# mehtas30/Software-Defined-Radio-Course-Project

Hardware: NVIDIA B200
Metric: input IQ Msamples/s (mode 0 stereo) (higher is better)
Workload: dtype f32

## Files before the change

### software-defined-radio-course-project_b200/csrc/fmrx_kernels.cu

```cuda
#include <cstddef>
#include <mutex>
#include <type_traits>

#include "fmrx_internal.h"
#ifdef FMRX_PLL_PROFILE
#include <cstdio>
#endif

namespace fmrx {

constexpr int kMaxDevices = 64;
struct DeviceCfg {
    size_t rf_smem[2][3] = {};
    size_t audio_smem = 0;
    size_t bp_smem = 0;
    size_t pll_ring_only = 0, pll_whole_sm = 0;
    int sm_count = 0;
};
static std::mutex g_cfg_mutex;
static DeviceCfg g_cfg[kMaxDevices];
static DeviceCfg *device_cfg()
{
    int dev = -1;
    if (cudaGetDevice(&dev) != cudaSuccess || dev < 0 || dev >= kMaxDevices)
// ... 722 lines not shown
        int2 v;
        asm volatile("ld.shared.v2.b32 {%0, %1}, [%2];" : "=r"(v.x), "=r"(v.y) : "r"(addr));
        return v;
    };
    auto load_half = [&](unsigned addr) {
        int4 v;
        asm volatile("ld.volatile.shared.v4.b32 {%0, %1, %2, %3}, [%4];" : "=r"(v.x), "=r"(v.y), "=r"(v.z), "=r"(v.w) : "r"(addr) : "memory");
        return v;
    };
    auto settle = [&](int u0, int nb, float integ0, float ph0, int gi0) -> bool {
        if (guards_failed()) {
#ifdef FMRX_PLL_PROFILE
            r.prof_stamp += bad != 0;
            r.prof_c += bad == 0;
            if (bad == 0) {
                if (!(cmax < 1e30f)) r.prof_inv++;
                else if (cmax > 0.5f) r.prof_range++;
                else r.prof_tie++;
            }
#endif
            r.kbase = kbase;
            r.integ = integ0;
            r.ph = ph0;
            r.gi = gi0;
            n_exact++;
            if (!pll_block_exact(r, u0, nb, lane)) {
#ifdef FMRX_PLL_PROFILE
                r.prof_fatal_exact++;
                if (blockIdx.x == 0 && lane == 0)
                    printf("pll dbg fatal: group base %d block at %d (of %d) gi %d kbase %d\n", base, u0 - base, cnt, r.gi, r.kbase);
                __syncwarp();
#endif
                return false;
            }
            integ = r.integ;
            ph = r.ph;
            kpe = r.kpe;
            kie = r.kie;
            gi = r.gi;
        }
        bad = 0;
        cmax = 0.0f;
        return true;
    };
    auto load_rec = [&](int u) {
        int2 v;
        asm volatile("ld.volatile.shared.v2.b32 {%0, %1}, [%2];" : "=r"(v.x), "=r"(v.y) : "r"(sph_base + (unsigned)(u & (PLL_PH_RING - 1)) * 8u) : "memory");
        return v;
    };
    float pi_next = 0.0f;
    int kbase_next = 0, seq_next = 0;
    auto next_pi = [&](int u0) {
        const bool have = seq_next == u0 && fabsf(pi_next) < 2097152.0f;
        pi_f = have ? pi_next : pi_f;
        kbase = have ? kbase_next : kbase;
        bad |= (int)!have;
    };
    int t = 0;
    int fatal = 0;
    const int n_full = cnt >> 4;
    if (r.cont) {
        const int2 rec = load_rec(base - 1);
        block_pi(__int_as_float(rec.x), inv_ulp_f, pi_next, kbase_next);
        seq_next = rec.y;
    } else {
        pi_next = pi_f;
        kbase_next = kbase;
        seq_next = base;
    }
    for (int b = 0; b < n_full; b++, t += 16) {
        const int u0 = base + t;
        next_pi(u0);
        asm volatile("st.shared.b32 [%0], %1;" ::"r"(kb_base + 4u * (unsigned)(t >> 4)), "r"(kbase) : "memory");
        const float integ0 = integ, ph0 = ph;
        const int gi0 = gi;
        integ = p_faddf(integ, kie);
        ph = p_faddf(ph, p_faddf(kpe, integ));
        const unsigned in_a0 = in_base + (unsigned)(u0 & (PLL_RING - 1)) * (unsigned)sizeof(PllIn);
        const unsigned tab_a0 = tab_base + (unsigned)(u0 & (PLL_TABLES - 1)) * (unsigned)sizeof(PllRow);
        const int stamp = pll_stamp(u0, kbase);
        int gis[16];
        int4 rb0 = load_half(tab_a0 + 16u), ra0 = load_half(tab_a0);
        int4 rb1 = load_half(tab_a0 + (unsigned)sizeof(PllRow) + 16u), ra1 = load_half(tab_a0 + (unsigned)sizeof(PllRow));
        const int2 vg_last = load_vg(in_a0 + 15u * (unsigned)sizeof(PllIn));
#pragma unroll
        for (int j = 0; j < 16; j++) {
            int4 rb2 = rb1, ra2 = ra1;
            if (j + 2 < 16) {
                rb2 = load_half(tab_a0 + (unsigned)(j + 2) * (unsigned)sizeof(PllRow) + 16u);
                ra2 = load_half(tab_a0 + (unsigned)(j + 2) * (unsigned)sizeof(PllRow));
            }
            gis[j] = step(ra0, rb0, stamp, j == 15);
            ra0 = ra1; rb0 = rb1;
            ra1 = ra2; rb1 = rb2;
            if (j == 8) {
                const int2 rec = load_rec(u0 + 15);
                block_pi(__int_as_float(rec.x), inv_ulp_f, pi_next, kbase_next);
                seq_next = rec.y;
            }
        }
        gi = vg_last.x + kbase + __float_as_int(p_faddf(p_faddf(__int_as_float(gis[15]), __int_as_float(vg_last.y)), 12582912.0f));
#pragma unroll
        for (int j = 0; j < 16; j += 4)
            asm volatile("st.shared.v4.b32 [%0], {%1, %2, %3, %4};" ::"r"(sg_base + 4u * (unsigned)(t + j)), "r"(gis[j]), "r"(gis[j + 1]),
                         "r"(gis[j + 2]), "r"(gis[j + 3])
                         : "memory");
        if (!settle(u0, 16, integ0, ph0, gi0)) {
            fatal = 2;
            break;
        }
        if (n_exact > PLL_EXACT_MAX) {
            fatal = 1;
            break;
        }
        asm volatile("st.volatile.shared.b32 [%0], %1;" ::"r"(prog_addr), "r"(u0 + 16) : "memory");
    }
    if (!fatal && t < cnt) {
        const int u0 = base + t, nb = cnt - t;
        next_pi(u0);
        asm volatile("st.shared.b32 [%0], %1;" ::"r"(kb_base + 4u * (unsigned)(t >> 4)), "r"(kbase) : "memory");
        const float integ0 = integ, ph0 = ph;
        const int gi0 = gi;
        integ = p_faddf(integ, kie);
        ph = p_faddf(ph, p_faddf(kpe, integ));
        for (int j = 0; j < nb; j++) {
            const int u = u0 + j;
            const unsigned row = tab_base + (unsigned)(u & (PLL_TABLES - 1)) * (unsigned)sizeof(PllRow);
            const int4 rb = load_half(row + 16u), ra = load_half(row);
            const int2 vg = load_vg(in_base + (unsigned)(u & (PLL_RING - 1)) * (unsigned)sizeof(PllIn));
            const int tb = step(ra, rb, pll_stamp(u0, kbase), j == nb - 1);
            gi = vg.x + kbase + __float_as_int(p_faddf(p_faddf(__int_as_float(tb), __int_as_float(vg.y)), 12582912.0f));
            asm volatile("st.shared.b32 [%0], %1;" ::"r"(sg_base + 4u * (unsigned)(t + j)), "r"(tb) : "memory");
        }
        fatal = settle(u0, nb, integ0, ph0, gi0) ? 0 : 2;
    }
    r.fatal = fatal;
    r.t_stop = t;
    r.n_exact = n_exact;
    if (fatal == 2)
        return;
    r.integ = integ;
    r.ph = ph;
    r.kpe = kpe;
    r.kie = kie;
    r.gi = gi;
}

__global__ void __launch_bounds__(PLL_THREADS) k_pll(const PllArgs a)
{
    using namespace pllcore;
    extern __shared__ __align__(16) unsigned char pll_dyn_smem[];
    PllIn *s_in = reinterpret_cast<PllIn *>(pll_dyn_smem);
    __shared__ __align__(16) int2 s_ph[PLL_PH_RING];
    __shared__ float s_hdr[3];
    __shared__ double s_hdr_tad;
    __shared__ int s_kbase;
    __shared__ int s_kb_blk[2][PLL_GROUP / 16];
    __shared__ int s_prog;
    __shared__ PllRow s_tab[PLL_TABLES];
    __shared__ __align__(16) int s_g[2][PLL_GROUP];
    __shared__ double s_grid[2];
    __shared__ double s_prep_ulp[2];
    __shared__ int s_head_ready[PLL_IO_WARPS];
    __shared__ double s_ulp_hist[2];
    __shared__ int s_spec[2];
    __shared__ int s_split[2];
    __shared__ int s_flag[5];
    __shared__ int s_redo;

    const int c = blockIdx.x;
    const int warp = threadIdx.x >> 5, lane = threadIdx.x & 31;
    const float *p = a.pilot + (size_t)c * a.pilot_stride;
    float *tr = a.trig + (size_t)c * a.if_stride + a.if_off;
    float *st = a.state + 8 * (size_t)c;
    const int n = a.n_if;

    Consts k;
    k.kp = a.prm.kp;
    k.ki = a.prm.ki;
    k.w = a.prm.w;
    const TrigK &K = a.kconst;

    const float toff0 = st[5];
    const bool regular = toff_is_regular(toff0);
    const int t0 = regular ? (int)toff0 : 0;
    const int role = warp & 3;
    const int io_id = warp >> 2;
    const int cand_id = (warp >> 2) * 2 + role - 2;

    auto prepare_one = [&](int u, float e_slope, float e_ph, int e_base) {
        {
            const float pvv = (u < n) ? p[u] : 1.0f;
            const float pnx = (u + 1 < n) ? p[u + 1] : 1.0f;
            PllIn in;
            in.x = pvv;
            in.inv_x = 1.0 / (double)pvv;
            const float toff = (float)min(t0 + u + 1, 16777216);
            in.v = __dmul_rn(k.w, (double)toff);
            const double qv = grid_round(in.v, s_grid[1]);
            in.vi = grid_index(qv);
            in.vr = __double2float_rn(__fma_rn(in.v, s_grid[1], -p_add(qv, -FMRX_RINT_MAGIC)));
            in.c3 = predictor_c(k, pvv, (float)min(t0 + u, 16777216));
            in.h1 = onehyp_inputs(in.v, e_ph, e_slope, u + 1 - e_base, pnx);
            s_in[u & (PLL_RING - 1)] = in;
        }
    };
    auto prepare = [&](int base, float e_slope, float e_ph, int e_base) {
        for (int j = 32 * io_id; j < PLL_GROUP; j += 32 * PLL_IO_WARPS)
            prepare_one(base + j + lane, e_slope, e_ph, e_base);
        if (lane == 0 && io_id == 0)
            s_prep_ulp[(base / PLL_GROUP) & 1] = s_grid[0];
    };
    auto head_ready = [&](int next_base) -> bool {
        for (int spin = 0; spin < PLL_SPIN_LIMIT; spin++) {
            int a0, a1;
            asm volatile("ld.volatile.shared.b32 %0, [%1];" : "=r"(a0) : "r"(smem_u32(&s_head_ready[0])) : "memory");
            asm volatile("ld.volatile.shared.b32 %0, [%1];" : "=r"(a1) : "r"(smem_u32(&s_head_ready[1])) : "memory");
            if (a0 == next_base && a1 == next_base)
                return true;
        }
        return false;
    };

    for (int i = threadIdx.x; i < PLL_PH_RING; i += PLL_THREADS)
        s_ph[i] = make_int2(0, 0);
    for (int i = threadIdx.x; i < PLL_TABLES; i += PLL_THREADS) {
        s_tab[i].lp = PLL_ROW_INVALID;
        s_tab[i].stamp = 0;
        s_tab[i].kie0 = 0.0f;
    }
    if (threadIdx.x == 0) {
        s_flag[1] = 0;
        s_redo = 0;
        s_head_ready[0] = s_head_ready[1] = -1;
    }
    Chain ch;
    bool stale = false;
    bool have_ed = false;
    float kpe_next = 0.0f, kie_next = 0.0f;
    bool dead = false;
    int backoff = 0, skip = 0;
    int prev_scheme = 0;
    float ph_hdr_prev = 0.0f;
    int n_groups = 0, n_redone = 0, n_exact = 0, prev_exact = 0;
    float pred_integ = 0.0f, pred_ph = 0.0f;
#ifdef FMRX_PLL_PROFILE
    long long prof_steps_cyc = 0, prof_wait = 0, prof_pre = 0, prof_one_cyc = 0;
    long long prof_t_end = 0, prof_bar2 = 0, prof_hdr = 0, prof_bar1 = 0, prof_post = 0, prof_post2 = 0, prof_c1 = 0;
    const long long prof_k0 = clock64();
    int prof_steps = 0, prof_n_stamp = 0, prof_n_c = 0, prof_n_fe = 0, prof_n_fm = 0;
    int prof_n_tie = 0, prof_n_range = 0, prof_n_inv = 0;
    int prof_one_steps = 0, prof_one_groups = 0, prof_one_exact = 0, prof_one_short = 0, prof_checked = 0;
    __shared__ int s_prof[8];
    __shared__ long long s_prof1[8];
    if (threadIdx.x < 8) {
        s_prof[threadIdx.x] = 0;
        s_prof1[threadIdx.x] = 0;
    }
#endif
    if (warp == 0) {
        ch.integ = st[0];
        ch.ph = st[1];
        ch.fi = st[2];
        ch.fq = st[3];
        ch.toff = toff0;
        chain_load(ch, k);
        if (lane == 0) {
            s_grid[0] = ch.ulp;
            s_grid[1] = ch.inv_ulp;
        }
    }
    __syncthreads();
    if (role == 1 && io_id < PLL_IO_WARPS) {
        prepare(0, st[0], st[1], 0);
    }
    __syncthreads();

    for (int base = 0, g = 0; base < n;) {
        const int cnt = min(PLL_GROUP, n - base);
        Chain ck;
#ifdef FMRX_PLL_PROFILE
        const long long prof_h0 = clock64();
        if (warp == 0 && prof_t_end)
            prof_bar2 += prof_h0 - prof_t_end;
#endif
        if (warp == 0) {
            ck = ch;
            const bool again = s_redo != 0;
            const bool usable = regular && !dead && ch.binade != FMRX_DISARMED && fabs(ch.tad) <= (double)FMRX_FAST_TRIG_MAX;
            const bool can3 = usable && !again && skip == 0 && (double)fabsf(ch.ph) < ch.ulp * 16777216.0;
            const bool regrid = can3 && s_prep_ulp[g & 1] != ch.ulp;
            const int scheme = can3 ? 3 : usable ? 1 : 0;
            const bool cont = scheme == 3 && prev_scheme == 3 && have_ed && prev_exact <= 2 && !regrid;
#ifdef FMRX_PLL_PROFILE
            prof_post += clock64() - prof_h0;
#endif
            if (scheme != prev_scheme || again) {
                for (int i = lane; i < PLL_TABLES; i += 32) {
                    s_tab[i].lp = PLL_ROW_INVALID;
                    s_tab[i].stamp = 0;
                    s_tab[i].kie0 = 0.0f;
                }
                for (int i = lane; i < PLL_PH_RING; i += 32)
                    s_ph[i] = make_int2(0, 0);
            } else if (scheme == 3 && !cont && base > 0) {
                for (int i = lane; i < PLL_HEAD; i += 32) {
                    s_tab[(base + i) & (PLL_TABLES - 1)].lp = PLL_ROW_INVALID;
                    s_tab[(base + i) & (PLL_TABLES - 1)].stamp = 0;
                    s_ph[(base + i) & (PLL_PH_RING - 1)] = make_int2(0, 0);
                }
            }
            if (lane == 0) {
                s_flag[0] = scheme;
                s_flag[2] = regrid;
                s_grid[0] = ch.ulp;
                s_grid[1] = ch.inv_ulp;
                s_flag[3] = cont;
                s_flag[4] = again;
                s_kbase = __float_as_int(p_faddf(p_fmulf(ch.ph, (float)ch.inv_ulp), 12582912.0f)) - 0x4B400000 - 0x4B400000;
                s_hdr[0] = ch.integ;
                s_hdr[1] = ch.ph;
                if (!again) {
                    s_hdr[2] = g > 0 ? p_fmulf(p_faddf(ch.ph, -ph_hdr_prev), 1.0f / PLL_GROUP) : ch.integ;
                    ph_hdr_prev = ch.ph;
                }
                s_hdr_tad = ch.tad;
                s_prog = base;
            }
        }
#ifdef FMRX_PLL_PROFILE
        const long long prof_h1 = clock64();
#endif
        __syncthreads();
#ifdef FMRX_PLL_PROFILE
        if (warp == 0) {
            prof_hdr += prof_h1 - prof_h0;
            prof_bar1 += clock64() - prof_h1;
        }
#endif
        if (s_flag[2]) {
            const double iu = s_grid[1];
            for (int j = threadIdx.x; j < PLL_GROUP; j += PLL_THREADS) {
                PllIn &in = s_in[(base + j) & (PLL_RING - 1)];
                const double qv = grid_round(in.v, iu);
                in.vi = grid_index(qv);
                in.vr = __double2float_rn(__fma_rn(in.v, iu, -p_add(qv, -FMRX_RINT_MAGIC)));
            }
            if (threadIdx.x == 0)
                s_prep_ulp[g & 1] = s_grid[0];
            __syncthreads();
        }
        const int scheme = s_flag[0];
        const bool spec = scheme == 3;
        const bool again = s_flag[4] != 0;
        const double ulp = s_grid[0], inv_ulp = s_grid[1];
#ifdef FMRX_PLL_PROFILE
        const long long prof_ga = clock64();
#endif

        if (warp == 0) {
            if (lane == 0)
                s_redo = 0;
            if (!again)
                n_groups++;
            bool good = scheme != 0;
            bool redo = false;
            bool regridded = false;
            int split = 0;
            int parked = 0;
            if (scheme == 3) {
                float integ = ch.integ, ph = ch.ph;
                float kpe = kpe_next, kie = kie_next;
                if (!have_ed) {
                    const PllIn i0 = s_in[base & (PLL_RING - 1)];
                    const Feedback f0 = make_feedback(K, ch.tad, pll_turn(i0.x), i0.inv_x, nullptr, nullptr);
                    const float ed = error_from_feedback(f0, i0.x, (double)i0.x, good);
                    kpe = p_fmulf(k.kp, ed);
                    kie = p_fmulf(k.ki, ed);
                }
                const float inv_ulp_f = (float)inv_ulp;
                float pi_f = 0.0f;
                int cu_base = 0;
                auto recentre = [&]() {
                    const float pm = p_faddf(p_fmulf(ph, inv_ulp_f), 12582912.0f);
                    pi_f = p_faddf(pm, -12582912.0f);
                    cu_base = __float_as_int(pm) - 0x4B400000 - 0x4B400000;
                    good &= fabsf(pi_f) < 2097152.0f;
                };
                recentre();
#ifdef FMRX_PLL_PROFILE
                const long long prof_w0 = clock64();
                prof_pre += prof_w0 - prof_ga;
#endif
                {
                    const bool need = lane < 16 && lane < cnt;
                    int spin = 0;
                    for (;;) {
                        const int z = ld_v4(&s_tab[(base + (lane & 15)) & (PLL_TABLES - 1)].kpe2).w;
                        if (__all_sync(0xffffffffu, !need || (z & 0x3ffffff) == base + 1) || ++spin >= PLL_SPIN_LIMIT)
                            break;
                    }
                    if (spin >= PLL_SPIN_LIMIT) {
                        dead = true;
                        good = false;
                        if (lane == 0)
                            s_flag[1] = 1;
                    }
                }
#ifdef FMRX_PLL_PROFILE
                prof_wait += clock64() - prof_w0;
#endif
                TableRun r;
                r.integ = integ;
                r.ph = ph;
                r.kpe = kpe;
                r.kie = kie;
                r.inv_ulp_f = inv_ulp_f;
                r.pi_f = pi_f;
                r.kbase = cu_base;
                r.base = base;
                r.cnt = cnt;
                r.in_base = smem_u32(&s_in[0]) + (unsigned)offsetof(PllIn, vi);
                r.tab_base = smem_u32(&s_tab[0]);
                r.sg_base = smem_u32(&s_g[g & 1][0]);
                r.prog_addr = smem_u32(&s_prog);
                r.sph_base = smem_u32(&s_ph[0]);
                r.kb_base = smem_u32(&s_kb_blk[g & 1][0]);
                r.head_addr = smem_u32(&s_head_ready[0]);
                r.cont = s_flag[3];
#ifdef FMRX_PLL_PROFILE
                r.prof_stamp = r.prof_c = r.prof_fatal_exact = 0;
                r.prof_tie = r.prof_range = r.prof_inv = 0;
#endif
                r.gi = __double2int_rn(p_mul(ch.tad, inv_ulp));
                r.n_exact = 0;
                r.fatal = 0;
                r.ring = s_in;
                r.k = k;
                r.ulp = ulp;
                r.toff_base = ch.toff;
                if (good) {
                    __syncwarp();
#ifdef FMRX_PLL_PROFILE
                    const long long prof_c0 = clock64();
#endif
                    pll_table_group(r, lane);
#ifdef FMRX_PLL_PROFILE
                    prof_c1 = clock64();
                    prof_steps_cyc += prof_c1 - prof_c0;
                    prof_steps += cnt;
                    prof_n_stamp += r.prof_stamp;
                    prof_n_c += r.prof_c;
                    prof_n_fe += r.prof_fatal_exact;
                    prof_n_tie += r.prof_tie;
                    prof_n_range += r.prof_range;
                    prof_n_inv += r.prof_inv;
                    prof_n_fm += r.fatal && !r.prof_fatal_exact;
#endif
                    good = r.fatal == 0;
                    n_exact += r.n_exact;
                    prev_exact = r.n_exact;
                }
                if (good && r.fatal == 0)
                    split = cnt;
                if (r.fatal == 2) {
                    asm volatile("st.volatile.shared.b32 [%0], %1;" ::"r"(smem_u32(&s_prog)), "r"(PLL_ABANDONED) : "memory");
                    split = r.t_stop;
                    onehyp_chain_at(ch, r.integ, r.ph, (float)min(t0 + base + r.t_stop, 16777216), p_mul((double)r.gi, ulp));
                    pll_group_checked(ch, k, s_in, base, r.t_stop, cnt, regular, smem_u32(&s_g[g & 1][0]), false);
                    stale = false;
                    have_ed = false;
                    parked = 1;
                    regridded = true;
                } else if (good) {
                    ch.integ = r.integ;
                    ch.ph = r.ph;
                    ch.toff = (float)min(t0 + base + cnt, 16777216);
                    ch.tad = p_mul((double)r.gi, ulp);
                    stale = true;
                    have_ed = true;
                    kpe_next = r.kpe;
                    kie_next = r.kie;
                    backoff = 0;
                    parked = 1;
                } else {
                    asm volatile("st.volatile.shared.b32 [%0], %1;" ::"r"(smem_u32(&s_prog)), "r"(PLL_ABANDONED) : "memory");
                    n_redone++;
                    backoff = min(backoff < 4 ? backoff + 1 : 2 * backoff, PLL_BACKOFF_MAX);
                    skip = backoff;
                    ch = ck;
                    have_ed = false;
                    redo = !dead;
                    if (!redo) {
                        if (stale) {
                            chain_refresh(ch);
                            stale = false;
                        }
                        pll_group_checked(ch, k, s_in, base, 0, cnt, regular, smem_u32(&s_g[g & 1][0]), false);
                    }
                }
            } else if (scheme == 1) {
                if (skip > 0 && !again)
                    skip--;
                OneRun r;
                r.integ = ch.integ;
                r.ph = ch.ph;
                r.base = base;
                r.cnt = cnt;
                r.tab_base = smem_u32(&s_tab[0]);
                r.sg_base = smem_u32(&s_g[g & 1][0]);
                r.prog_addr = smem_u32(&s_prog);
                r.ring = s_in;
                r.k = k;
                r.toff_base = ch.toff;
                r.tad0 = ch.tad;
                r.n_exact = 0;
                r.done = 0;
                r.timed_out = 0;
                __syncwarp();
#ifdef FMRX_PLL_PROFILE
                const long long prof_c0 = clock64();
#endif
                pll_onehyp_group(r, lane);
#ifdef FMRX_PLL_PROFILE
                prof_one_cyc += clock64() - prof_c0;
                prof_one_steps += r.done;
                prof_one_groups++;
                prof_one_exact += r.n_exact;
                prof_one_short += r.done < cnt;
#endif
                n_exact += r.n_exact;
                if (r.timed_out) {
                    dead = true;
                    if (lane == 0)
                        s_flag[1] = 1;
                }
                const int last = base + r.done - 1;
                const double tad = r.done ? onehyp_trigarg(s_in[last & (PLL_RING - 1)].v, r.ph) : ch.tad;
                if (r.done < cnt) {
                    asm volatile("st.volatile.shared.b32 [%0], %1;" ::"r"(smem_u32(&s_prog)), "r"(PLL_ABANDONED) : "memory");
                    onehyp_chain_at(ch, r.integ, r.ph, (float)min(t0 + base + r.done, 16777216), tad);
                    pll_group_checked(ch, k, s_in, base, r.done, cnt, regular, smem_u32(&s_g[g & 1][0]), true);
                    stale = false;
                } else {
                    ch.integ = r.integ;
                    ch.ph = r.ph;
                    ch.toff = (float)min(t0 + base + cnt, 16777216);
                    ch.tad = tad;
                    stale = true;
                    if (fabs(tad) <= (double)FMRX_FAST_TRIG_MAX)
                        chain_arm(ch);
                    else
                        onehyp_chain_at(ch, r.integ, r.ph, ch.toff, tad), stale = false;
                }
                have_ed = false;
                parked = 2;
            } else {
                if (skip > 0)
                    skip--;
                if (stale) {
                    chain_refresh(ch);
                    stale = false;
                }
#ifdef FMRX_PLL_PROFILE
                prof_checked++;
#endif
                pll_group_checked(ch, k, s_in, base, 0, cnt, regular, smem_u32(&s_g[g & 1][0]), false);
                have_ed = false;
                parked = 0;
            }
            prev_scheme = redo || regridded ? 0 : scheme;
            if (lane == 0) {
                s_spec[g & 1] = parked;
                s_split[g & 1] = split;
                s_ulp_hist[g & 1] = ulp;
                s_redo = redo;
            }
#ifdef FMRX_PLL_PROFILE
            prof_t_end = clock64();
            if (prof_c1)
                prof_post2 += prof_t_end - prof_c1;
            prof_c1 = 0;
#endif
        } else if (role >= 2) {
            if (scheme == 3) {
                const int sq = lane >> 2, jq = lane & 3;
                const unsigned prog_a = smem_u32(&s_prog);
                auto progress = [&]() {
                    int v;
                    asm volatile("ld.volatile.shared.b32 %0, [%1];" : "=r"(v) : "r"(prog_a) : "memory");
                    return v;
                };
                const bool cont = s_flag[3] != 0;
                const int first = base + (cont ? PLL_HEAD : 0);
                const int end = base + cnt + (base + cnt + PLL_HEAD <= n ? PLL_HEAD : 0);
                const int q0 = first / PLL_BATCH;
                bool head_seen = false;
                for (int ub8 = first + ((cand_id - q0 % PLL_CAND_WARPS + PLL_CAND_WARPS) % PLL_CAND_WARPS) * PLL_BATCH; ub8 < end;
                     ub8 += PLL_BATCH * PLL_CAND_WARPS) {
                    if (!head_seen && cnt == PLL_GROUP && ub8 + PLL_BATCH >= base + cnt) {
                        if (!head_ready(base + PLL_GROUP)) {
                            s_flag[1] = 1;
                            break;
                        }
                        head_seen = true;
                    }
                    const bool live = ub8 + sq < end;
                    const int u = ub8 + (live ? sq : 0);
                    const double v = s_in[u & (PLL_RING - 1)].v;
                    const int vi = s_in[u & (PLL_RING - 1)].vi;
                    const float vr = s_in[u & (PLL_RING - 1)].vr;
                    const PllIn nx = s_in[(u + 1) & (PLL_RING - 1)];
                    const int last = min(ub8 + PLL_BATCH - 1, end - 1);
                    int prog = 0, spin = 0;
                    for (;; spin++) {
                        const int seq = ld_v2(&s_ph[last & (PLL_PH_RING - 1)]).y;
                        if (seq - (last + 1) >= 0 || spin >= PLL_SPIN_LIMIT)
                            break;
                        if ((spin & 7) == 7 && (prog = progress()) == PLL_ABANDONED)
                            break;
                    }
                    if (prog == PLL_ABANDONED)
                        break;
                    if (spin >= PLL_SPIN_LIMIT) {
                        s_flag[1] = 1;
                        break;
                    }
                    const int2 pr = ld_v2(&s_ph[u & (PLL_PH_RING - 1)]);
                    const int ub = ub8 & ~15;
                    int kb = s_kbase;
                    bool have_pi = true;
                    if (ub != base || cont) {
                        const int2 rb = ld_v2(&s_ph[(ub - 1) & (PLL_PH_RING - 1)]);
                        float pif;
                        block_pi(__int_as_float(rb.x), (float)inv_ulp, pif, kb);
                        have_pi = rb.y == ub;
                    }
                    const bool have = pr.y == u + 1 && have_pi;
                    const int gc = grid_index(grid_round(p_add(v, (double)__int_as_float(pr.x)), inv_ulp));
                    const int gl = gc - 1 + jq;
                    const double tad = p_mul((double)gl, ulp);
                    const Feedback f = make_feedback(K, tad, pll_turn(nx.x), nx.inv_x, nullptr, nullptr);
                    const int ag = gl < 0 ? -gl : gl;
                    bool ok = have && ag > (1 << 23) && ag < (1 << 24);
#ifdef FMRX_PLL_PROFILE
                    const bool prof_ok_b = ok;
#endif
                    const float ed = error_from_feedback(f, nx.x, (double)nx.x, ok);
                    const int n1 = gc - (vi + kb) - 0x4B400000;
#ifdef FMRX_PLL_PROFILE
                    if (live && jq < 3 && blockIdx.x == 0) {
                        if (!(pr.y == u + 1)) atomicAdd(&s_prof[0], 1);
                        else if (!have_pi) atomicAdd(&s_prof[1], 1);
                        else if (!prof_ok_b) atomicAdd(&s_prof[2], 1);
                        else if (!ok) atomicAdd(&s_prof[fabs(f.phi) >= FMRX_SEAM_PHI_MAX ? 3 : 4], 1);
                        else if (!(n1 >= -60 && n1 <= 60)) atomicAdd(&s_prof[5], 1);
                        else atomicAdd(&s_prof[6], 1);
                    }
#endif
                    ok = ok && n1 >= -60 && n1 <= 60;
                    const unsigned oks = __ballot_sync(0xffffffffu, ok || jq == 3);
                    const bool valid = ((oks >> (4 * sq)) & 7u) == 7u;
                    for (spin = 0; (prog = progress()) != PLL_ABANDONED && prog - (ub8 + PLL_BATCH - PLL_TABLES) < 0 && spin < PLL_SPIN_LIMIT;
                         spin++)
                        ;
                    if (prog == PLL_ABANDONED)
                        break;
                    if (spin >= PLL_SPIN_LIMIT) {
                        s_flag[1] = 1;
                        break;
                    }
                    if (live && prog - (ub8 + PLL_BATCH) < 0) {
                        const int lo = jq < 3 ? __float_as_int(p_fmulf(k.kp, ed))
                                              : __float_as_int(valid ? p_faddf(p_faddf((float)n1, -0.5f), -vr) : PLL_ROW_INVALID);
                        const int hi = jq < 3 ? __float_as_int(p_fmulf(k.ki, ed)) : pll_stamp(u & ~15, kb);
                        asm volatile("st.volatile.shared.v2.b32 [%0], {%1, %2};" ::"r"(smem_u32(&s_tab[u & (PLL_TABLES - 1)]) + 8u * (unsigned)jq),
                                     "r"(lo), "r"(hi)
                                     : "memory");
                    }
                }
            } else if (scheme == 1) {
                const unsigned prog_a = smem_u32(&s_prog);
                auto progress = [&]() {
                    int v;
                    asm volatile("ld.volatile.shared.b32 %0, [%1];" : "=r"(v) : "r"(prog_a) : "memory");
                    return v;
                };
                const int end = base + cnt;
                for (int ub = base + cand_id * PLL_BATCH1; ub < end; ub += PLL_BATCH1 * PLL_CAND_WARPS) {
                    const bool live = ub + lane < end;
                    const int u = live ? ub + lane : end - 1;
                    const int last = min(ub + PLL_BATCH1 - 1, end - 1);
                    int prog = 0, spin = 0;
#ifdef FMRX_PLL_PROFILE
                    const long long cw0 = clock64();
#endif
                    for (;; spin++) {
                        const int seq = ld_v2(&s_ph[last & (PLL_PH_RING - 1)]).y;
                        if (seq == last + 1 || spin >= PLL_SPIN_LIMIT)
                            break;
                        if ((spin & 7) == 7 && (prog = progress()) == PLL_ABANDONED)
                            break;
                    }
                    if (prog == PLL_ABANDONED)
                        break;
                    if (spin >= PLL_SPIN_LIMIT) {
                        s_flag[1] = 1;
                        break;
                    }
#ifdef FMRX_PLL_PROFILE
                    const long long cw1 = clock64();
#endif
                    const int2 cur = ld_v2(&s_ph[u & (PLL_PH_RING - 1)]);
                    bool ok = cur.y == u + 1;
                    double tad = s_hdr_tad;
                    if (u != base) {
                        const int2 prv = ld_v2(&s_ph[(u - 1) & (PLL_PH_RING - 1)]);
                        ok = ok && prv.y == u;
                        tad = onehyp_trigarg(s_in[(u - 1) & (PLL_RING - 1)].v, __int_as_float(prv.x));
                    }
                    const float x = s_in[u & (PLL_RING - 1)].x;
                    const double inv_x = s_in[u & (PLL_RING - 1)].inv_x;
                    ok = ok && fabs(tad) <= (double)FMRX_FAST_TRIG_MAX;
                    const Feedback f = make_feedback(K, ok ? tad : 0.0, pll_turn(x), inv_x, nullptr, nullptr);
                    const float ed = error_from_feedback(f, x, (double)x, ok);
                    for (spin = 0; (prog = progress()) != PLL_ABANDONED && prog - (ub + PLL_BATCH1 - PLL_TABLES1) < 0 && spin < PLL_SPIN_LIMIT; spin++)
                        ;
                    if (prog == PLL_ABANDONED)
                        break;
                    if (spin >= PLL_SPIN_LIMIT) {
                        s_flag[1] = 1;
                        break;
                    }
                    if (live)
                        st_v4(reinterpret_cast<PllRow1 *>(&s_tab[0]) + (u & (PLL_TABLES1 - 1)), __float_as_int(p_fmulf(k.kp, ed)),
                              __float_as_int(p_fmulf(k.ki, ed)), cur.x, ok ? u + 1 : -(u + 1));
#ifdef FMRX_PLL_PROFILE
                    if (lane == 0 && blockIdx.x == 0 && cand_id == 0) {
                        s_prof1[3] += clock64() - cw1;
                        s_prof1[4] += 1;
                        s_prof1[5] += cw1 - cw0;
                    }
#endif
                }
            }
        } else if (warp == PLL_PRED_WARP) {
            if (scheme == 3) {
                const bool cont = s_flag[3] != 0;
                if (!cont) {
                    pred_integ = s_hdr[0];
                    pred_ph = s_hdr[1];
                }
                float integ = pred_integ, ph = pred_ph;
                const unsigned prog_a = smem_u32(&s_prog);
                const unsigned ph_a = smem_u32(&s_ph[0]);
                const unsigned c_a = smem_u32(&s_in[0]) + (unsigned)offsetof(PllIn, c3);
                int prog = base;
                const int t_end = cnt + (base + cnt + PLL_HEAD <= n ? PLL_HEAD : 0);
                for (int t = cont ? PLL_HEAD : 0; t < t_end; t += 16) {
                    const int u0 = base + t;
                    if (t == PLL_GROUP && !head_ready(base + PLL_GROUP)) {
                        s_flag[1] = 1;
                        break;
                    }
                    int spin = 0;
                    do {
                        asm volatile("ld.volatile.shared.b32 %0, [%1];" : "=r"(prog) : "r"(prog_a) : "memory");
                    } while (prog != PLL_ABANDONED && u0 - prog > PLL_PRED_LEAD - 16 && ++spin < PLL_SPIN_LIMIT);
                    if (prog == PLL_ABANDONED || spin >= PLL_SPIN_LIMIT)
                        break;
                    const unsigned c_a0 = c_a + (unsigned)(u0 & (PLL_RING - 1)) * (unsigned)sizeof(PllIn);
                    const unsigned ph_a0 = ph_a + (unsigned)(u0 & (PLL_PH_RING - 1)) * 8u;
                    float cs[16];
#pragma unroll
                    for (int j = 0; j < 16; j++)
                        asm volatile("ld.shared.b32 %0, [%1];" : "=f"(cs[j]) : "r"(c_a0 + (unsigned)j * (unsigned)sizeof(PllIn)));
#pragma unroll
                    for (int j = 0; j < 16; j++) {
                        predictor_step(k, cs[j], integ, ph);
                        asm volatile("st.volatile.shared.v2.b32 [%0], {%1, %2};" ::"r"(ph_a0 + (unsigned)j * 8u), "r"(__float_as_int(ph)),
                                     "r"(u0 + j + 1)
                                     : "memory");
                    }
                }
                pred_integ = integ;
                pred_ph = ph;
            } else if (scheme == 1) {
                float integ = s_hdr[0], ph = s_hdr[1];
                float ang = onehyp_first_angle(s_in[base & (PLL_RING - 1)].x, s_hdr_tad);
                int careful = 0;
                const unsigned prog_a = smem_u32(&s_prog);
                const unsigned ph_a = smem_u32(&s_ph[0]);
                const unsigned h_a = smem_u32(&s_in[0]) + (unsigned)offsetof(PllIn, h1);
                const bool short_form = onehyp_short_ok(s_hdr_tad, s_hdr[1]);

                int prog = base;
                for (int t = 0; t < cnt; t += PLL_PBLK) {
                    const int u0 = base + t;
                    int spin = 0;
#ifdef FMRX_PLL_PROFILE
                    const long long pw0 = clock64();
#endif
                    while (prog != PLL_ABANDONED && u0 - prog > PLL_LEAD1 - PLL_PBLK && ++spin < PLL_SPIN_LIMIT)
                        asm volatile("ld.volatile.shared.b32 %0, [%1];" : "=r"(prog) : "r"(prog_a) : "memory");
#ifdef FMRX_PLL_PROFILE
                    const long long pw1 = clock64();
                    if (lane == 0 && blockIdx.x == 0)
                        s_prof1[0] += pw1 - pw0;
#endif
                    if (prog == PLL_ABANDONED || spin >= PLL_SPIN_LIMIT)
                        break;
                    int prog_next;
                    asm volatile("ld.volatile.shared.b32 %0, [%1];" : "=r"(prog_next) : "r"(prog_a) : "memory");
                    const unsigned h_a0 = h_a + (unsigned)(u0 & (PLL_RING - 1)) * (unsigned)sizeof(PllIn);
                    const unsigned ph_a0 = ph_a + (unsigned)(u0 & (PLL_PH_RING - 1)) * 8u;
                    OneHypIn hs[PLL_PBLK];
#pragma unroll
                    for (int j = 0; j < PLL_PBLK; j++)
                        asm volatile("ld.shared.v4.f32 {%0, %1, %2, %3}, [%4];"
                                     : "=f"(hs[j].P), "=f"(hs[j].r), "=f"(hs[j].B), "=f"(hs[j].c)
                                     : "r"(h_a0 + (unsigned)j * (unsigned)sizeof(PllIn)));
                    const float ang0 = ang, integ0 = integ, ph0 = ph;
                    float phs[PLL_PBLK];
                    bool reduce = careful > 0;
                    if (!reduce) {
                        float amax = fabsf(ang);
                        if (short_form) {
                            float crs[PLL_PBLK];
#pragma unroll
                            for (int j = 0; j < PLL_PBLK; j++)
                                crs[j] = p_faddf(hs[j].c, -hs[j].r);
#pragma unroll
                            for (int j = 0; j < PLL_PBLK; j++) {
                                ang = onehyp_predictor_step_short(k, hs[j].P, crs[j], ang, integ, ph);
                                phs[j] = ph;
                                if (j < PLL_PBLK - 1)
                                    amax = fmaxf(amax, fabsf(ang));
                            }
                        } else {
#pragma unroll
                            for (int j = 0; j < PLL_PBLK; j++) {
                                ang = onehyp_predictor_step(k, hs[j], ang, integ, ph);
                                phs[j] = ph;
                                if (j < PLL_PBLK - 1)
                                    amax = fmaxf(amax, fabsf(ang));
                            }
                        }
                        reduce = !(amax <= FMRX_ONEHYP_PI);
                        if (reduce)
                            careful = 8;
                    } else {
                        careful--;
                    }
                    if (reduce) {
                        ang = ang0;
                        integ = integ0;
                        ph = ph0;
                        if (!(fabsf(ang) <= FMRX_ONEHYP_PI))
                            ang = p_faddf(ang, -p_fmulf(6.2831855f, p_faddf(p_faddf(p_fmulf(ang, 0.15915494f), 12582912.0f), -12582912.0f)));
#pragma unroll
                        for (int j = 0; j < PLL_PBLK; j++) {
                            ang = onehyp_predictor_step_reduced(k, hs[j], ang, integ, ph);
                            phs[j] = ph;
                        }
                    }
#pragma unroll
                    for (int j = 0; j < PLL_PBLK; j++)
                        asm volatile("st.volatile.shared.v2.b32 [%0], {%1, %2};" ::"r"(ph_a0 + (unsigned)j * 8u), "r"(__float_as_int(phs[j])),
                                     "r"(u0 + j + 1)
                                     : "memory");
#ifdef FMRX_PLL_PROFILE
                    if (lane == 0 && blockIdx.x == 0) {
                        s_prof1[1] += clock64() - pw1;
                        s_prof1[2] += reduce;
                    }
#endif
                    prog = prog_next;
                }
            }
        } else if (role == 1 && io_id < PLL_IO_WARPS) {
            if (!again) {
                const int pb = base - PLL_GROUP, pg = (g - 1) & 1;
                const int kind_g = g > 0 ? s_spec[pg] : 0, split = g > 0 ? s_split[pg] : 0;
                for (int j = lane + 32 * io_id; j < PLL_GROUP; j += 32 * PLL_IO_WARPS) {
                    if (g > 0) {
                        const PllIn &in = s_in[(pb + j) & (PLL_RING - 1)];
                        const int w = s_g[pg][j];
                        const int kind = kind_g == 1 && j >= split ? 0 : kind_g;
                        tr[pb + j] = kind == 1   ? __double2float_rn(p_mul((double)parked_index(w, in, s_kb_blk[pg][j >> 4]), s_ulp_hist[pg]))
                                     : kind == 2 ? __double2float_rn(onehyp_trigarg(in.v, __int_as_float(w)))
                                                 : __int_as_float(w);
                    }
                    prepare_one(base + PLL_GROUP + j, s_hdr[2], s_hdr[1], base);
                    if (j < 32 * PLL_IO_WARPS) {
                        __syncwarp();
                        if (lane == 0) {
                            __threadfence_block();
                            asm volatile("st.volatile.shared.b32 [%0], %1;" ::"r"(smem_u32(&s_head_ready[io_id])), "r"(base + PLL_GROUP) : "memory");
                        }
                    }
                }
                if (lane == 0 && io_id == 0)
                    s_prep_ulp[(g + 1) & 1] = s_grid[0];
            }
        }
        __syncthreads();
        if (!s_redo) {
            base += PLL_GROUP;
            g++;
        }
    }
    if (warp == 1 && n > 0) {
        const int g = (n - 1) / PLL_GROUP, pb = g * PLL_GROUP, pg = g & 1;
        const int kind_g = s_spec[pg], split = s_split[pg];
        for (int j = lane; pb + j < n && j < PLL_GROUP; j += 32) {
            const PllIn &in = s_in[(pb + j) & (PLL_RING - 1)];
            const int w = s_g[pg][j];
            const int kind = kind_g == 1 && j >= split ? 0 : kind_g;
            tr[pb + j] = kind == 1   ? __double2float_rn(p_mul((double)parked_index(w, in, s_kb_blk[pg][j >> 4]), s_ulp_hist[pg]))
                         : kind == 2 ? __double2float_rn(onehyp_trigarg(in.v, __int_as_float(w)))
                                     : __int_as_float(w);
        }
    }
    if (warp == 0 && lane == 0) {
        if (stale)
            chain_refresh(ch);
        float fi, fq;
        chain_feedback(ch, fi, fq);
        st[0] = ch.integ;
        st[1] = ch.ph;
        st[2] = fi;
        st[3] = fq;
        st[5] = ch.toff;
#ifdef FMRX_PLL_PROFILE
        if (c == 0)
            printf("pll dbg why: blocks near a tie %d, grid point not among the three %d, no valid table %d | candidate lanes: record late %d, no block pi %d, binade edge %d, phi at the seam %d, cross/dot %d, |n1| > 60 %d, ok %d\n",
                   prof_n_tie, prof_n_range, prof_n_inv, s_prof[0], s_prof[1], s_prof[2], s_prof[3], s_prof[4], s_prof[5], s_prof[6]);
        if (c == 0)
            printf("pll dbg: groups %d exact blocks %d (stamp/pi %d, guard %d) redone %d (exact step left the grid %d, too many exact blocks %d) | %.1f cyc/step over %d table steps | kernel %.1f cyc/step; per group: before wait %.0f, wait for tables %.0f, steps %.0f, rest %.0f\n",
                   n_groups, n_exact, prof_n_stamp, prof_n_c, n_redone, prof_n_fe, prof_n_fm, prof_steps ? (double)prof_steps_cyc / prof_steps : 0.0, prof_steps, (double)(clock64() - prof_k0) / n,
                   (double)prof_pre / n_groups, (double)prof_wait / n_groups, (double)prof_steps_cyc / n_groups,
                   (double)(clock64() - prof_k0 - prof_pre - prof_wait - prof_steps_cyc) / n_groups);
        if (c == 0)
            printf("pll dbg group overhead (cycles per group, warp 0): waiting at the end-of-group barrier %.0f, header %.0f (its decisions %.0f), waiting at the header barrier %.0f, after the table steps %.0f\n",
                   (double)prof_bar2 / n_groups, (double)prof_hdr / n_groups, (double)prof_post / n_groups, (double)prof_bar1 / n_groups, (double)prof_post2 / n_groups);
        if (c == 0)
            printf("pll dbg one-hypothesis: groups %d (cut short %d), %.1f cyc/step over %d steps, exact blocks %d | groups without tables %d | predictor: %.1f cyc/step stepping, %.1f waiting for warp 0, %lld blocks of 8 reduced | candidate warp 2: %lld passes, %.0f cyc each, %.0f waiting for records\n",
                   prof_one_groups, prof_one_short, prof_one_steps ? (double)prof_one_cyc / prof_one_steps : 0.0, prof_one_steps, prof_one_exact, prof_checked,
                   prof_one_steps ? (double)s_prof1[1] / prof_one_steps : 0.0, prof_one_steps ? (double)s_prof1[0] / prof_one_steps : 0.0, s_prof1[2],
                   s_prof1[4], s_prof1[4] ? (double)s_prof1[3] / s_prof1[4] : 0.0, s_prof1[4] ? (double)s_prof1[5] / s_prof1[4] : 0.0);
#endif
        st[6] = (float)(n_groups + 1000 * min(n_exact, 999));
        st[7] = s_flag[1] ? -1.0f : (float)n_redone;
        if (n > 0)
            st[4] = nco_from_trig(__double2float_rn(ch.tad), a.prm.scale, a.prm.adjust);
    }
}

cudaError_t launch_pll(const PllArgs &a_in, int n_captures, cudaStream_t s)
{
    PllArgs a = a_in;
    a.kconst = pllcore::trig_constants();
    DeviceCfg *cfg = device_cfg();
    if (!cfg)
        return cudaErrorInvalidDevice;
    size_t ring_only, whole_sm;
    int sm_count;
    {
        std::lock_guard<std::mutex> lock(g_cfg_mutex);
        if (cfg->pll_ring_only == 0) {
            int dev = 0, optin = 0, sms = 0;
            cudaFuncAttributes fa;
            cudaError_t e = cudaGetDevice(&dev);
            if (e == cudaSuccess)
                e = cudaDeviceGetAttribute(&optin, cudaDevAttrMaxSharedMemoryPerBlockOptin, dev);
            if (e == cudaSuccess)
                e = cudaDeviceGetAttribute(&sms, cudaDevAttrMultiProcessorCount, dev);
            if (e == cudaSuccess)
                e = cudaFuncGetAttributes(&fa, k_pll);
            if (e != cudaSuccess)
                return e;
            const size_t need = sizeof(PllIn) * PLL_RING;
            size_t all = (size_t)optin > fa.sharedSizeBytes ? (size_t)optin - fa.sharedSizeBytes : 0;
            if (all < need)
                all = need;
            e = cudaFuncSetAttribute(k_pll, cudaFuncAttributeMaxDynamicSharedMemorySize, (int)all);
            if (e != cudaSuccess)
                return e;
            cfg->pll_whole_sm = all;
            cfg->pll_ring_only = need;
            cfg->sm_count = sms;
        }
        ring_only = cfg->pll_ring_only;
        whole_sm = cfg->pll_whole_sm;
        sm_count = cfg->sm_count;
    }
    const bool isolate = n_captures + kPllSpareSms <= sm_count;
    k_pll<<<n_captures, PLL_THREADS, isolate ? whole_sm : ring_only, s>>>(a);
    return cudaGetLastError();
}


__global__ void __launch_bounds__(kAudioTile) k_audio(const AudioArgs a, const int span)
{
    extern __shared__ float smem[];
    const int T = a.T, U = a.U, D = a.D, B = a.if_per_block, NA = a.audio_per_block;
    float *s_dem = smem;
    float *s_mix = s_dem + span;
    float *s_tail = s_mix + span;
    float *s_mono = s_tail + T;
    float *s_cf = s_mono + kAudioTile + kMonoDelay;

    const int c = blockIdx.y, tid = threadIdx.x;
    const int tiles_per_block = NA / kAudioTile;
    const int b_local = blockIdx.x / tiles_per_block;
    const int n_lo = (blockIdx.x % tiles_per_block) * kAudioTile;

    const size_t cap = (size_t)c * a.if_stride;
    const long long blk0 = (long long)a.if_off + (long long)b_local * B;
    const float *demod = a.demod + cap;
    const float *chan = a.chan + cap;
    const float *trig = a.trig + cap;

    const int q_first = (n_lo >= kMonoDelay) ? ((n_lo - kMonoDelay) * D) / U
                                             : ((NA - kMonoDelay) * D) / U - B;
    const int r_min = q_first - (T - 1);
    const int r_max = (n_lo + kAudioTile >= NA) ? B - 1 : ((n_lo + kAudioTile - 1) * D) / U;
    const int own_lo = n_lo ? ((n_lo - 1) * D) / U + 1 : 0;
    const int own_hi = r_max + 1;
    const int q_lo = (n_lo * D) / U;
    const int count = r_max - r_min + 1;

    for (int i = tid; i < count; i += kAudioTile) {
        const int r = r_min + i;
        const long long g = blk0 + r;
        const float ch = chan[g];
        const float nco = nco_from_trig(trig[g], a.scale, a.adjust);
        const float mx = mix2(ch, nco);
        s_dem[i] = demod[g];
        s_mix[i] = mx;
        if (a.nco && r >= own_lo && r < own_hi) {
            const size_t sg = (size_t)c * a.if_stage_stride + a.if_stage_off + (size_t)b_local * B + r;
            a.nco[sg] = nco;
            a.mixer[sg] = mx;
        }
    }
    const bool need_tail = (q_lo - (T - 1)) < 0;
    if (need_tail)
        for (int i = tid; i < T - 1; i += kAudioTile)
            s_tail[i] = demod[blk0 + B - (T - 1) + i];
    if (U == 1)
        for (int i = tid; i < T; i += kAudioTile)
            s_cf[i] = a.coef_pm[i];
    __syncthreads();

    const int n = n_lo + tid;
    float am = 0.0f, as = 0.0f;
    {
        const int nd = n * D;
        const int q = nd / U;
        const float *cf = U == 1 ? s_cf : a.coef_pm + (size_t)(nd % U) * T;
        const int t_in = min(T, q + 1);
        const float *xd = s_dem + (q - r_min), *xm = s_mix + (q - r_min);
// ... 291 lines not shown
```

Before: 26060.

## Skip per-group header barrier when PLL continues in steady-state table scheme

At the end of each group, the chain warp now computes whether the next group will be a continuing scheme-3 group. It publishes the IO warps' header values into a double-buffered slot, so the next iteration can skip the header setup phase and its __syncthreads. This cuts one block-wide barrier and the header bookkeeping per group on the serial PLL critical path. In exchange, the duplicated eligibility logic must stay consistent with the original scheme selection, and table invalidation is skipped on the fast path.

```diff
diff --git a/software-defined-radio-course-project_b200/csrc/fmrx_kernels.cu b/software-defined-radio-course-project_b200/csrc/fmrx_kernels.cu
--- a/software-defined-radio-course-project_b200/csrc/fmrx_kernels.cu
+++ b/software-defined-radio-course-project_b200/csrc/fmrx_kernels.cu
@@ -898,7 +898,9 @@
     extern __shared__ __align__(16) unsigned char pll_dyn_smem[];
     PllIn *s_in = reinterpret_cast<PllIn *>(pll_dyn_smem);
     __shared__ __align__(16) int2 s_ph[PLL_PH_RING];
-    __shared__ float s_hdr[3];
+    __shared__ float s_hdr[2];
+    __shared__ float s_io_hdr[2][2];
+    __shared__ int s_next_cont;
     __shared__ double s_hdr_tad;
     __shared__ int s_kbase;
     __shared__ int s_kb_blk[2][PLL_GROUP / 16];
@@ -1022,83 +1024,96 @@
     }
     __syncthreads();
 
+    bool fast = false;
     for (int base = 0, g = 0; base < n;) {
         const int cnt = min(PLL_GROUP, n - base);
         Chain ck;
-#ifdef FMRX_PLL_PROFILE
-        const long long prof_h0 = clock64();
-        if (warp == 0 && prof_t_end)
-            prof_bar2 += prof_h0 - prof_t_end;
-#endif
-        if (warp == 0) {
+        if (!fast) {
+#ifdef FMRX_PLL_PROFILE
+            const long long prof_h0 = clock64();
+            if (warp == 0 && prof_t_end)
+                prof_bar2 += prof_h0 - prof_t_end;
+#endif
+            if (warp == 0) {
+                ck = ch;
+                const bool again = s_redo != 0;
+                const bool usable = regular && !dead && ch.binade != FMRX_DISARMED && fabs(ch.tad) <= (double)FMRX_FAST_TRIG_MAX;
+                const bool can3 = usable && !again && skip == 0 && (double)fabsf(ch.ph) < ch.ulp * 16777216.0;
+                const bool regrid = can3 && s_prep_ulp[g & 1] != ch.ulp;
+                const int scheme = can3 ? 3 : usable ? 1 : 0;
+                const bool cont = scheme == 3 && prev_scheme == 3 && have_ed && prev_exact <= 2 && !regrid;
+#ifdef FMRX_PLL_PROFILE
+                prof_post += clock64() - prof_h0;
+#endif
+                if (scheme != prev_scheme || again) {
+                    for (int i = lane; i < PLL_TABLES; i += 32) {
+                        s_tab[i].lp = PLL_ROW_INVALID;
+                        s_tab[i].stamp = 0;
+                        s_tab[i].kie0 = 0.0f;
+                    }
+                    for (int i = lane; i < PLL_PH_RING; i += 32)
+                        s_ph[i] = make_int2(0, 0);
+                } else if (scheme == 3 && !cont && base > 0) {
+                    for (int i = lane; i < PLL_HEAD; i += 32) {
+                        s_tab[(base + i) & (PLL_TABLES - 1)].lp = PLL_ROW_INVALID;
+                        s_tab[(base + i) & (PLL_TABLES - 1)].stamp = 0;
+                        s_ph[(base + i) & (PLL_PH_RING - 1)] = make_int2(0, 0);
+                    }
+                }
+                if (lane == 0) {
+                    s_flag[0] = scheme;
+                    s_flag[2] = regrid;
+                    s_grid[0] = ch.ulp;
+                    s_grid[1] = ch.inv_ulp;
+                    s_flag[3] = cont;
+                    s_flag[4] = again;
+                    s_kbase = __float_as_int(p_faddf(p_fmulf(ch.ph, (float)ch.inv_ulp), 12582912.0f)) - 0x4B400000 - 0x4B400000;
+                    s_hdr[0] = ch.integ;
+                    s_hdr[1] = ch.ph;
+                    if (!again) {
+                        s_io_hdr[g & 1][0] = ch.ph;
+                        s_io_hdr[g & 1][1] = g > 0 ? p_fmulf(p_faddf(ch.ph, -ph_hdr_prev), 1.0f / PLL_GROUP) : ch.integ;
+                        ph_hdr_prev = ch.ph;
+                    }
+                    s_hdr_tad = ch.tad;
+                    s_prog = base;
+                }
+            }
+#ifdef FMRX_PLL_PROFILE
+            const long long prof_h1 = clock64();
+#endif
+            __syncthreads();
+#ifdef FMRX_PLL_PROFILE
+            if (warp == 0) {
+                prof_hdr += prof_h1 - prof_h0;
+                prof_bar1 += clock64() - prof_h1;
+            }
+#endif
+            if (s_flag[2]) {
+                const double iu = s_grid[1];
+                for (int j = threadIdx.x; j < PLL_GROUP; j += PLL_THREADS) {
+                    PllIn &in = s_in[(base + j) & (PLL_RING - 1)];
+                    const double qv = grid_round(in.v, iu);
+                    in.vi = grid_index(qv);
+                    in.vr = __double2float_rn(__fma_rn(in.v, iu, -p_add(qv, -FMRX_RINT_MAGIC)));
+                }
+                if (threadIdx.x == 0)
+                    s_prep_ulp[g & 1] = s_grid[0];
+                __syncthreads();
+            }
+        } else if (warp == 0) {
             ck = ch;
-            const bool again = s_redo != 0;
-            const bool usable = regular && !dead && ch.binade != FMRX_DISARMED && fabs(ch.tad) <= (double)FMRX_FAST_TRIG_MAX;
-            const bool can3 = usable && !again && skip == 0 && (double)fabsf(ch.ph) < ch.ulp * 16777216.0;
-            const bool regrid = can3 && s_prep_ulp[g & 1] != ch.ulp;
-            const int scheme = can3 ? 3 : usable ? 1 : 0;
-            const bool cont = scheme == 3 && prev_scheme == 3 && have_ed && prev_exact <= 2 && !regrid;
-#ifdef FMRX_PLL_PROFILE
-            prof_post += clock64() - prof_h0;
-#endif
-            if (scheme != prev_scheme || again) {
-                for (int i = lane; i < PLL_TABLES; i += 32) {
-                    s_tab[i].lp = PLL_ROW_INVALID;
-                    s_tab[i].stamp = 0;
-                    s_tab[i].kie0 = 0.0f;
-                }
-                for (int i = lane; i < PLL_PH_RING; i += 32)
-                    s_ph[i] = make_int2(0, 0);
-            } else if (scheme == 3 && !cont && base > 0) {
-                for (int i = lane; i < PLL_HEAD; i += 32) {
-                    s_tab[(base + i) & (PLL_TABLES - 1)].lp = PLL_ROW_INVALID;
-                    s_tab[(base + i) & (PLL_TABLES - 1)].stamp = 0;
-                    s_ph[(base + i) & (PLL_PH_RING - 1)] = make_int2(0, 0);
-                }
-            }
-            if (lane == 0) {
-                s_flag[0] = scheme;
-                s_flag[2] = regrid;
-                s_grid[0] = ch.ulp;
-                s_grid[1] = ch.inv_ulp;
-                s_flag[3] = cont;
-                s_flag[4] = again;
-                s_kbase = __float_as_int(p_faddf(p_fmulf(ch.ph, (float)ch.inv_ulp), 12582912.0f)) - 0x4B400000 - 0x4B400000;
-                s_hdr[0] = ch.integ;
-                s_hdr[1] = ch.ph;
-                if (!again) {
-                    s_hdr[2] = g > 0 ? p_fmulf(p_faddf(ch.ph, -ph_hdr_prev), 1.0f / PLL_GROUP) : ch.integ;
-                    ph_hdr_prev = ch.ph;
-                }
-                s_hdr_tad = ch.tad;
-                s_prog = base;
-            }
-        }
-#ifdef FMRX_PLL_PROFILE
-        const long long prof_h1 = clock64();
-#endif
-        __syncthreads();
-#ifdef FMRX_PLL_PROFILE
-        if (warp == 0) {
-            prof_hdr += prof_h1 - prof_h0;
-            prof_bar1 += clock64() - prof_h1;
-        }
-#endif
-        if (s_flag[2]) {
-            const double iu = s_grid[1];
-            for (int j = threadIdx.x; j < PLL_GROUP; j += PLL_THREADS) {
-                PllIn &in = s_in[(base + j) & (PLL_RING - 1)];
-                const double qv = grid_round(in.v, iu);
-                in.vi = grid_index(qv);
-                in.vr = __double2float_rn(__fma_rn(in.v, iu, -p_add(qv, -FMRX_RINT_MAGIC)));
-            }
-            if (threadIdx.x == 0)
-                s_prep_ulp[g & 1] = s_grid[0];
-            __syncthreads();
-        }
-        const int scheme = s_flag[0];
+            if (lane == 0)
+                ph_hdr_prev = ch.ph;
+#ifdef FMRX_PLL_PROFILE
+            if (prof_t_end)
+                prof_bar2 += clock64() - prof_t_end;
+#endif
+        }
+        const int scheme = fast ? 3 : s_flag[0];
         const bool spec = scheme == 3;
-        const bool again = s_flag[4] != 0;
+        const bool again = !fast && s_flag[4] != 0;
+        const bool cont = fast || s_flag[3] != 0;
         const double ulp = s_grid[0], inv_ulp = s_grid[1];
 #ifdef FMRX_PLL_PROFILE
         const long long prof_ga = clock64();
@@ -1173,7 +1188,7 @@
                 r.sph_base = smem_u32(&s_ph[0]);
                 r.kb_base = smem_u32(&s_kb_blk[g & 1][0]);
                 r.head_addr = smem_u32(&s_head_ready[0]);
-                r.cont = s_flag[3];
+                r.cont = cont;
 #ifdef FMRX_PLL_PROFILE
                 r.prof_stamp = r.prof_c = r.prof_fatal_exact = 0;
                 r.prof_tie = r.prof_range = r.prof_inv = 0;
@@ -1316,7 +1331,15 @@
                 parked = 0;
             }
             prev_scheme = redo || regridded ? 0 : scheme;
+            const bool next_cont = scheme == 3 && good && !redo && !regridded && have_ed && prev_exact <= 2 && skip == 0 && regular && !dead &&
+                                   ch.binade != FMRX_DISARMED && fabs(ch.tad) <= (double)FMRX_FAST_TRIG_MAX &&
+                                   (double)fabsf(ch.ph) < ch.ulp * 16777216.0;
             if (lane == 0) {
+                s_next_cont = next_cont;
+                if (next_cont) {
+                    s_io_hdr[(g + 1) & 1][0] = ch.ph;
+                    s_io_hdr[(g + 1) & 1][1] = p_fmulf(p_faddf(ch.ph, -ph_hdr_prev), 1.0f / PLL_GROUP);
+                }
                 s_spec[g & 1] = parked;
                 s_split[g & 1] = split;
                 s_ulp_hist[g & 1] = ulp;
@@ -1337,7 +1360,6 @@
                     asm volatile("ld.volatile.shared.b32 %0, [%1];" : "=r"(v) : "r"(prog_a) : "memory");
                     return v;
                 };
-                const bool cont = s_flag[3] != 0;
                 const int first = base + (cont ? PLL_HEAD : 0);
                 const int end = base + cnt + (base + cnt + PLL_HEAD <= n ? PLL_HEAD : 0);
                 const int q0 = first / PLL_BATCH;
@@ -1492,7 +1514,6 @@
             }
         } else if (warp == PLL_PRED_WARP) {
             if (scheme == 3) {
-                const bool cont = s_flag[3] != 0;
                 if (!cont) {
                     pred_integ = s_hdr[0];
                     pred_ph = s_hdr[1];
@@ -1637,7 +1658,7 @@
                                      : kind == 2 ? __double2float_rn(onehyp_trigarg(in.v, __int_as_float(w)))
                                                  : __int_as_float(w);
                     }
-                    prepare_one(base + PLL_GROUP + j, s_hdr[2], s_hdr[1], base);
+                    prepare_one(base + PLL_GROUP + j, s_io_hdr[g & 1][1], s_io_hdr[g & 1][0], base);
                     if (j < 32 * PLL_IO_WARPS) {
                         __syncwarp();
                         if (lane == 0) {
@@ -1655,6 +1676,7 @@
             base += PLL_GROUP;
             g++;
         }
+        fast = s_next_cont != 0 && s_prep_ulp[g & 1] == s_grid[0];
     }
     if (warp == 1 && n > 0) {
         const int g = (n - 1) / PLL_GROUP, pb = g * PLL_GROUP, pg = g & 1;
```

New measurement: 25950 (median of 6 runs). No clear change (-0.4%).
